# tryolabs/luminoth

Measured on NVIDIA H100. Metric: images/sec, higher is better.
Workload: dtype f32 (fp16x2-split operands on fp16 wgmma, fp32 accumulate)

## Files before the change

luminoth_b200/csrc/conv.cu:

```cuda
#include "conv.cuh"
#include <algorithm>
#include <cmath>
#include <cstdlib>
#include <cstring>
#include <map>
#include <mutex>
#include <tuple>

namespace lumi {

thread_local int g_launch_count = 0;

struct SimtArgs {
  const __half* in_hi; const __half* in_lo;
  int n, h, w, cin;
  const float* wgt; const float* scale; const float* bias;
  int kh, kw, stride, rate, pad_t, pad_l, ho, wo, cout, act;
  __half* out_hi; __half* out_lo; float* out_f32;
  const __half* res_hi; const __half* res_lo; int res_h, res_w, res_stride;
  int* overflow;
  const float* pre_scale; const float* pre_bias; __half* pre_hi; __half* pre_lo;
};

constexpr int SM_BM = 128, SM_BN = 64, SM_BK = 16;
// ... 131 lines not shown
        }
      }
    }
  }
}

void launch_conv_simt(const ConvLayer& L, const ConvIO& io, cudaStream_t st) {
  SimtArgs a;
  a.in_hi = io.in.hi; a.in_lo = io.in.lo;
  a.n = io.in.n; a.h = io.in.h; a.w = io.in.w; a.cin = io.in.c;
  LUMI_REQUIRE(io.in.c == L.cin, "conv_simt: channel mismatch");
  a.wgt = L.w_f32; a.scale = L.scale; a.bias = L.bias;
  a.kh = L.kh; a.kw = L.kw; a.stride = L.stride; a.rate = L.rate;
  a.pad_t = io.pad_t; a.pad_l = io.pad_l; a.ho = io.ho; a.wo = io.wo; a.cout = L.cout; a.act = L.act;
  a.out_hi = io.out.hi; a.out_lo = io.out.lo; a.out_f32 = io.out_f32;
  a.res_hi = io.res.hi; a.res_lo = io.res.lo; a.res_h = io.res.h; a.res_w = io.res.w; a.res_stride = io.res_stride;
  a.overflow = io.overflow_flag;
  a.pre_scale = io.pre_scale; a.pre_bias = io.pre_bias; a.pre_hi = io.pre.hi; a.pre_lo = io.pre.lo;
  LUMI_REQUIRE(!io.pre.hi || (!io.out_f32 && io.pre_scale && io.pre_bias), "conv_simt: bad pre-activation output");
  long M = (long)a.n * a.ho * a.wo;
  if (M == 0) return;
  dim3 grid((unsigned)cdiv64(M, SM_BM), (unsigned)cdiv(L.cout, SM_BN));
  if (io.pre.hi) conv_simt_kernel<true><<<grid, 256, 0, st>>>(a);
  else conv_simt_kernel<false><<<grid, 256, 0, st>>>(a);
  count_launch();
  LUMI_CUDA_CHECK(cudaGetLastError());
}

struct TcArgs {
  CUtensorMap tm_a_hi, tm_a_lo, tm_b_hi, tm_b_lo;
  CUtensorMap tm_o_hi, tm_o_lo, tm_r_hi, tm_r_lo;
  CUtensorMap tm_p_hi, tm_p_lo;
  const float* pre_scale; const float* pre_bias;
  __half* pre_hi; __half* pre_lo;
  const float* scale; const float* bias;
  __half* out_hi; __half* out_lo; float* out_f32;
  const __half* res_hi; const __half* res_lo;
  int res_h, res_w, res_stride;
  int n, ho, wo, cin, cout;
  int kh, kw, rate, pad_t, pad_l, act;
  int nb, th, tw;
  int tiles_w, tiles_h, tiles_n;
  int n_tiles;
  int stride;
  int* overflow;
  int sk_mode;
  float* sk_partials;
  int* sk_flags;
  int sk_epoch;
};

struct TcItem { int tile, k0, k1; };
struct TcSched {
  int mode, total_tiles, n_iters, t, bid, nblk;
  long long u, u_end;
  __device__ TcSched(int mode_, int total_tiles_, int n_iters_, int bid_, int nblk_)
      : mode(mode_), total_tiles(total_tiles_), n_iters(n_iters_), bid(bid_), nblk(nblk_) {
    t = bid;
    const long long U = (long long)total_tiles * n_iters;
    u = U * bid / nblk;
    u_end = U * (bid + 1) / nblk;
  }
  __device__ static long long range_end(int unit, int total_tiles, int n_iters, int nblk_) {
    return (long long)total_tiles * n_iters * (unit + 1) / nblk_;
  }
  __device__ bool next(TcItem& it) {
    if (!mode) {
      if (t >= total_tiles) return false;
      it.tile = t; it.k0 = 0; it.k1 = n_iters;
      t += nblk;
      return true;
    }
    if (u >= u_end) return false;
    it.tile = (int)(u / n_iters);
    it.k0 = (int)(u - (long long)it.tile * n_iters);
    const long long rem = u_end - u;
    it.k1 = (rem < (long long)(n_iters - it.k0)) ? it.k0 + (int)rem : n_iters;
    u += it.k1 - it.k0;
    return true;
  }
};

constexpr int TC_A_BYTES = 128 * 128;
constexpr int TC_HALO_TW = 8;
constexpr int TC_HALO_PITCH = 2048;
constexpr int TC_HALO_ROWS = 16 + 2;
constexpr int TC_HALO_PLANE_BYTES = TC_HALO_ROWS * TC_HALO_PITCH;

template <int BN, int STAGES, int NCWG = 2, bool PAIR = false, bool HALO = false, int SLOTS = 0>
struct TcCfg {
  static_assert(NCWG == 2 || NCWG == 4, "two or four consumer warpgroups");
  static_assert(!PAIR || BN == 128, "the cluster pair exists for BN = 128");
  static constexpr int WN = BN * 2 / NCWG;
  static_assert(SLOTS == 0 || (!PAIR && !HALO && WN % 64 == 0), "slot epilogue: generic kernel, whole column groups");
  static_assert(NCWG == 2 || SLOTS % 2 == 0, "four warpgroups: an even slot count");
  static constexpr int B_BYTES = BN * 128;
  static constexpr int A_STAGE_BYTES = HALO ? 0 : 2 * TC_A_BYTES;
  static constexpr int STAGE_BYTES = A_STAGE_BYTES + 2 * B_BYTES;
  static constexpr int PATCH_BYTES = HALO ? 2 * TC_HALO_PLANE_BYTES : 0;
  static constexpr int SLOT_BYTES = 2 * TC_A_BYTES;
  static constexpr int SMEM_BYTES = 2 * PATCH_BYTES + STAGES * STAGE_BYTES + SLOTS * SLOT_BYTES + 1024  +
                                    256 ;
  static_assert(SMEM_BYTES <= 232448, "shared memory per CTA");
  static constexpr int THREADS = (1 + NCWG) * 128;
  static constexpr int LAUNCH_REGS = (65536 / THREADS) / 8 * 8;
  static constexpr int PRODUCER_REGS = NCWG == 2 ? 40 : 24;
  static constexpr int CONSUMER_REGS = NCWG == 2 ? 232 : 112;
  static_assert(128 * (PRODUCER_REGS + NCWG * CONSUMER_REGS) <= THREADS * LAUNCH_REGS, "register budget of the CTA");
};

struct TcSlice { uint64_t ahi, alo, bhi, blo; uint32_t st, pb; };

template <int WN>
__device__ __forceinline__ void tc_slice_mma(float (&d)[WN / 2], const TcSlice& s) {
  wgmma_fence();
#pragma unroll
  for (int kk = 0; kk < 4; ++kk) {
    const uint64_t ko = (uint64_t)(kk * 2);
    if constexpr (WN == 128) {
      wgmma_m64n128k16_f16(d, s.ahi + ko, s.blo + ko, kk > 0 ? 1u : 0u);
      wgmma_m64n128k16_f16(d, s.alo + ko, s.bhi + ko, 1u);
    } else {
      wgmma_m64n64k16_f16(d, s.ahi + ko, s.blo + ko, kk > 0 ? 1u : 0u);
      wgmma_m64n64k16_f16(d, s.alo + ko, s.bhi + ko, 1u);
    }
  }
#pragma unroll
  for (int kk = 0; kk < 4; ++kk) {
    const uint64_t ko = (uint64_t)(kk * 2);
    if constexpr (WN == 128) wgmma_m64n128k16_f16(d, s.ahi + ko, s.bhi + ko, 1u);
    else wgmma_m64n64k16_f16(d, s.ahi + ko, s.bhi + ko, 1u);
  }
  wgmma_commit();
}

__device__ __forceinline__ bool tc_preact(__half2& h2, __half2& l2, const float* s, const float* b, int c0) {
  const float2 sc = __ldg(reinterpret_cast<const float2*>(s + c0));
  const float2 bi = __ldg(reinterpret_cast<const float2*>(b + c0));
  const float p0 = fmaxf(fmaf(__low2float(h2) + __low2float(l2), sc.x, bi.x), 0.f);
  const float p1 = fmaxf(fmaf(__high2float(h2) + __high2float(l2), sc.y, bi.y), 0.f);
  split2_f32(p0, p1, h2, l2);
  return split_overflows(p0) || split_overflows(p1);
}

template <int BN, int STAGES, int NCWG, bool PAIR, bool HALO, bool PIPE, int SLOTS, bool PRE>
__global__ void __launch_bounds__(TcCfg<BN, STAGES, NCWG, PAIR, HALO, SLOTS>::THREADS, 1)
conv_tc_kernel(const __grid_constant__ TcArgs a) {
  using Cfg = TcCfg<BN, STAGES, NCWG, PAIR, HALO, SLOTS>;
  static_assert(!PRE || !HALO, "pre-activation outputs: generic and 2-CTA kernels");
  constexpr int WN = Cfg::WN;
  constexpr int NR = WN / 2;
  constexpr int NGT = BN / 64;
  extern __shared__ uint8_t smem_raw[];
  uint8_t* smem = smem_raw + ((1024u - (smem_u32(smem_raw) & 1023u)) & 1023u);
  uint8_t* patch = smem;
  uint8_t* stages = smem + 2 * Cfg::PATCH_BYTES;
  uint8_t* slots = stages + STAGES * Cfg::STAGE_BYTES;
  uint64_t* full_bar = reinterpret_cast<uint64_t*>(slots + SLOTS * Cfg::SLOT_BYTES);
  uint64_t* empty_bar = full_bar + STAGES;
  uint64_t* patch_full_bar = empty_bar + STAGES;
  uint64_t* patch_empty_bar = patch_full_bar + 2;
  uint64_t* slot_full_bar = patch_empty_bar + 2;
  uint64_t* slot_empty_bar = slot_full_bar + SLOTS;

  const int rank = PAIR ? (int)cluster_ctarank() : 0;
  const int sched_id = PAIR ? (int)(blockIdx.x >> 1) : (int)blockIdx.x;
  const int sched_n = PAIR ? (int)(gridDim.x >> 1) : (int)gridDim.x;
  const int wg = threadIdx.x >> 7;
  const int m_tiles = a.tiles_w * a.tiles_h * a.tiles_n;
  const int total_tiles = (PAIR ? (m_tiles + 1) / 2 : m_tiles) * a.n_tiles;
  const int rows_valid = a.nb * a.th * a.tw;
  const int cchunks = a.cin >> 6;
  const int n_iters = a.kh * a.kw * cchunks;

  if (threadIdx.x == 0) {
    for (int s = 0; s < STAGES; ++s) { mbar_init(&full_bar[s], 1); mbar_init(&empty_bar[s], (PAIR ? 2 : 1) * NCWG); }
    for (int s = 0; s < 2; ++s) { mbar_init(&patch_full_bar[s], 1); mbar_init(&patch_empty_bar[s], NCWG); }
    for (int s = 0; s < SLOTS; ++s) { mbar_init(&slot_full_bar[s], 1); mbar_init(&slot_empty_bar[s], 1); }
    fence_mbar_init();
    tma_prefetch_desc(&a.tm_a_hi); tma_prefetch_desc(&a.tm_a_lo);
    tma_prefetch_desc(&a.tm_b_hi); tma_prefetch_desc(&a.tm_b_lo);
    if (SLOTS) {
      tma_prefetch_desc(&a.tm_o_hi); tma_prefetch_desc(&a.tm_o_lo);
      if (a.res_hi) { tma_prefetch_desc(&a.tm_r_hi); tma_prefetch_desc(&a.tm_r_lo); }
      if (PRE && a.out_hi) { tma_prefetch_desc(&a.tm_p_hi); tma_prefetch_desc(&a.tm_p_lo); }
    }
  }
  if (PAIR) cluster_sync_all();
  else __syncthreads();

  if (wg == 0) {
    setmaxnreg_dec<Cfg::PRODUCER_REGS>();
    if (threadIdx.x == 0) {
      const uint32_t stage_tx = (HALO ? 0u : 2u * (uint32_t)rows_valid * 128u) + 2u * (uint32_t)Cfg::B_BYTES;
      const uint32_t patch_tx = 2u * (uint32_t)(a.th + 2) * (uint32_t)((TC_HALO_TW + 2) * 128);
      const uint32_t res_tx = 2u * (uint32_t)rows_valid * 128u;
      uint32_t git = 0, gpatch = 0, gslot = 0;
      TcSched sched(a.sk_mode, total_tiles, n_iters, sched_id, sched_n);
      TcItem item;
      while (sched.next(item)) {
        const int t = item.tile;
        const int nt = t % a.n_tiles, mt = PAIR ? 2 * (t / a.n_tiles) + rank : t / a.n_tiles;
        const int x0 = (mt % a.tiles_w) * a.tw, y0 = ((mt / a.tiles_w) % a.tiles_h) * a.th;
        const int img0 = (mt / (a.tiles_w * a.tiles_h)) * a.nb, n0 = nt * BN;
        int patch_cc = -1;
        for (int k = item.k0; k < item.k1; ++k, ++git) {
          const int tap = HALO ? k % 9 : k / cchunks, cc = HALO ? k / 9 : k - tap * cchunks;
          const int r = tap / a.kw, s = tap % a.kw;
          const int iy = y0 * a.stride + r * a.rate - a.pad_t, ix = x0 * a.stride + s * a.rate - a.pad_l;
          if (HALO && cc != patch_cc) {
            patch_cc = cc;
            const uint32_t pb = gpatch & 1u;
            mbar_wait(&patch_empty_bar[pb], ((gpatch >> 1) & 1u) ^ 1u);
            uint8_t* pbase = patch + pb * Cfg::PATCH_BYTES;
            mbar_arrive_expect_tx(&patch_full_bar[pb], patch_tx);
            for (int i = 0; i < a.th + 2; ++i) {
              tma_load_4d(pbase + i * TC_HALO_PITCH, &a.tm_a_hi, &patch_full_bar[pb], cc * 64, x0 - a.pad_l,
                          y0 - a.pad_t + i, img0);
              tma_load_4d(pbase + TC_HALO_PLANE_BYTES + i * TC_HALO_PITCH, &a.tm_a_lo, &patch_full_bar[pb], cc * 64,
                          x0 - a.pad_l, y0 - a.pad_t + i, img0);
            }
            ++gpatch;
          }
          const uint32_t st = git % STAGES, ph = (git / STAGES) & 1u;
          mbar_wait(&empty_bar[st], ph ^ 1u);
          uint8_t* sbase = stages + st * Cfg::STAGE_BYTES;
          const int kcol = tap * a.cin + cc * 64;
          mbar_arrive_expect_tx(&full_bar[st], stage_tx);
          if (!HALO) {
            tma_load_4d(sbase, &a.tm_a_hi, &full_bar[st], cc * 64, ix, iy, img0);
            tma_load_4d(sbase + TC_A_BYTES, &a.tm_a_lo, &full_bar[st], cc * 64, ix, iy, img0);
          }
// ... 7 lines not shown
            tma_load_2d(bbase + Cfg::B_BYTES, &a.tm_b_lo, &full_bar[st], kcol, n0);
          }
        }
        if constexpr (SLOTS > 0) {
          for (int g = 0; g < NGT && item.k0 == 0; ++g, ++gslot) {
            const uint32_t sl = gslot % SLOTS;
            mbar_wait(&slot_empty_bar[sl], ((gslot / SLOTS) & 1u) ^ 1u);
            if (a.res_hi) {
              uint8_t* sb = slots + sl * Cfg::SLOT_BYTES;
              mbar_arrive_expect_tx(&slot_full_bar[sl], res_tx);
              tma_load_4d(sb, &a.tm_r_hi, &slot_full_bar[sl], n0 + g * 64, x0 * a.res_stride, y0 * a.res_stride, img0);
              tma_load_4d(sb + TC_A_BYTES, &a.tm_r_lo, &slot_full_bar[sl], n0 + g * 64, x0 * a.res_stride,
                          y0 * a.res_stride, img0);
            } else {
              mbar_arrive(&slot_full_bar[sl]);
            }
          }
        }
      }
    }
  } else {
    setmaxnreg_inc<Cfg::CONSUMER_REGS>();
    const int c = wg - 1;
    const int ctid = threadIdx.x - 128;
    const int wrow = (c & 1) * 64, wcol = (c >> 1) * WN;
    const int lrow = ((threadIdx.x & 127) >> 5) * 16 + ((threadIdx.x & 31) >> 2);
    const int lcol = 2 * (threadIdx.x & 3);
    uint32_t git = 0, gpatch = 0;
    uint32_t gslot = 0, rel = 0;
    const bool slot_issuer = (threadIdx.x & 127) == 0 && (c & 1) == 0;
    TcSched sched(a.sk_mode, total_tiles, n_iters, sched_id, sched_n);
    TcItem item;
    while (sched.next(item)) {
      const int t = item.tile;
      const int nt = t % a.n_tiles, mt = PAIR ? 2 * (t / a.n_tiles) + rank : t / a.n_tiles;
      const int x0 = (mt % a.tiles_w) * a.tw, y0 = ((mt / a.tiles_w) % a.tiles_h) * a.th;
      const int img0 = (mt / (a.tiles_w * a.tiles_h)) * a.nb;
      const int n0 = nt * BN + wcol;

      float racc[NR];
#pragma unroll
      for (int j = 0; j < NR; ++j) racc[j] = 0.f;
      int patch_cc = -1;
      uint32_t pb = 0;
      auto acquire = [&](int k, uint32_t g) {
        TcSlice s;
        s.st = g % STAGES;
        if (HALO) {
          const int cc = k / 9, tap = k - cc * 9;
          if (cc != patch_cc) {
            patch_cc = cc;
            pb = gpatch & 1u;
            mbar_wait(&patch_full_bar[pb], (gpatch >> 1) & 1u);
            ++gpatch;
          }
          const int r = tap / 3, c3 = tap - r * 3;
          const uint32_t pa = smem_u32(patch + pb * Cfg::PATCH_BYTES) + (uint32_t)(((wrow >> 3) + r) * TC_HALO_PITCH + c3 * 128);
          s.ahi = make_sw128_kmajor_desc(pa, TC_HALO_PITCH);
          s.alo = make_sw128_kmajor_desc(pa + TC_HALO_PLANE_BYTES, TC_HALO_PITCH);
        }
        s.pb = pb;
        mbar_wait(&full_bar[s.st], (g / STAGES) & 1u);
        const uint32_t sa = smem_u32(stages + s.st * Cfg::STAGE_BYTES);
        if (!HALO) {
          s.ahi = make_sw128_kmajor_desc(sa + wrow * 128);
          s.alo = make_sw128_kmajor_desc(sa + TC_A_BYTES + wrow * 128);
        }
        s.bhi = make_sw128_kmajor_desc(sa + Cfg::A_STAGE_BYTES + wcol * 128);
        s.blo = make_sw128_kmajor_desc(sa + Cfg::A_STAGE_BYTES + Cfg::B_BYTES + wcol * 128);
        return s;
      };
      auto release = [&](int k, const TcSlice& s) {
        if ((threadIdx.x & 127) == 0) {
          mbar_arrive(&empty_bar[s.st]);
          if (PAIR) mbar_arrive_cluster(&empty_bar[s.st], (uint32_t)(rank ^ 1));
          if (HALO && (k + 1 == item.k1 || (k + 1) % 9 == 0)) mbar_arrive(&patch_empty_bar[s.pb]);
        }
      };
      auto fold = [&](float (&d)[NR]) {
        wgmma_fence_operand(d);
#pragma unroll
        for (int j = 0; j < NR; ++j) racc[j] = __fadd_rn(racc[j], d[j]);
      };
      if constexpr (PIPE) {
        const int k1 = item.k1;
        int k = item.k0;
        float d0[NR], d1[NR];
        TcSlice s0 = acquire(k, git), s1;
        tc_slice_mma<WN>(d0, s0);
        for (; k + 2 < k1; k += 2, git += 2) {
          s1 = acquire(k + 1, git + 1);
          tc_slice_mma<WN>(d1, s1);
          wgmma_wait1();
          release(k, s0);
          fold(d0);
          s0 = acquire(k + 2, git + 2);
          tc_slice_mma<WN>(d0, s0);
          wgmma_wait1();
          release(k + 1, s1);
          fold(d1);
        }
        if (k + 1 < k1) {
          s1 = acquire(k + 1, git + 1);
          tc_slice_mma<WN>(d1, s1);
          wgmma_wait1();
          release(k, s0);
          fold(d0);
          wgmma_wait0();
          release(k + 1, s1);
          fold(d1);
          git += 2;
        } else {
          wgmma_wait0();
          release(k, s0);
          fold(d0);
          git += 1;
        }
      } else {
        for (int k = item.k0; k < item.k1; ++k, ++git) {
          const TcSlice s = acquire(k, git);
          float d[NR];
          tc_slice_mma<WN>(d, s);
          wgmma_wait0();
          release(k, s);
          fold(d);
        }
      }

      if (item.k0 != 0) {
        float* wsp = a.sk_partials + (size_t)blockIdx.x * (128 * BN);
#pragma unroll
        for (int j = 0; j < NR; ++j) {
          const int row = wrow + lrow + ((j & 2) ? 8 : 0), col = wcol + (j >> 2) * 8 + lcol + (j & 1);
          wsp[col * 128 + row] = racc[j];
        }
        __threadfence();
        named_bar_sync(1, 128 * NCWG);
        if (ctid == 0)
          asm volatile("st.release.gpu.global.s32 [%0], %1;" ::"l"(a.sk_flags + blockIdx.x), "r"(a.sk_epoch) : "memory");
        continue;
      }
      if (item.k1 != n_iters) {
        const long long tile_end = (long long)(item.tile + 1) * n_iters;
        int last_unit = sched_id;
        for (int unit = sched_id + 1;; ++unit) {
          const int cta = PAIR ? 2 * unit + rank : unit;
          int seen;
          do {
            asm volatile("ld.acquire.gpu.global.s32 %0, [%1];" : "=r"(seen) : "l"(a.sk_flags + cta) : "memory");
          } while (seen != a.sk_epoch);
          const float* wsp = a.sk_partials + (size_t)cta * (128 * BN);
#pragma unroll
          for (int j = 0; j < NR; ++j) {
            const int row = wrow + lrow + ((j & 2) ? 8 : 0), col = wcol + (j >> 2) * 8 + lcol + (j & 1);
            racc[j] = __fadd_rn(racc[j], __ldcg(wsp + col * 128 + row));
          }
          last_unit = unit;
          if (TcSched::range_end(unit, total_tiles, n_iters, sched_n) >= tile_end) break;
        }
        named_bar_sync(1, 128 * NCWG);
        if (ctid == 0)
          for (int unit = sched_id + 1; unit <= last_unit; ++unit)
            asm volatile("st.relaxed.gpu.global.s32 [%0], %1;" ::"l"(a.sk_flags + (PAIR ? 2 * unit + rank : unit)), "r"(0) : "memory");
      }

      if constexpr (SLOTS > 0) {
        bool row_ok[2];
// ... 210 lines not shown
struct MapKey {
  const void* p; int a, b, c, d, e, f, g, kind;
  bool operator<(const MapKey& o) const {
    return std::tie(p, a, b, c, d, e, f, g, kind) < std::tie(o.p, o.a, o.b, o.c, o.d, o.e, o.f, o.g, o.kind);
  }
};
static std::map<MapKey, CUtensorMap> g_map_cache;
static std::mutex g_map_mutex;

static CUtensorMap cached_act_map(const __half* base, int n, int h, int w, int c, int nb, int th, int tw, int stride,
                                  long pix_pitch, long row_pitch, long img_pitch, MapKind kind = MAP_LOAD) {
  std::lock_guard<std::mutex> lk(g_map_mutex);
  MapKey k{base, n, h, w, c + (int)(pix_pitch << 12), nb, th * 16 + stride, tw, kind};
  auto it = g_map_cache.find(k);
  if (it != g_map_cache.end()) return it->second;
  if (g_map_cache.size() > 4096) g_map_cache.clear();
  CUtensorMap m = make_map_act(base, n, h, w, c, nb, th, tw, stride, pix_pitch, row_pitch, img_pitch);
  g_map_cache[k] = m;
  return m;
}
static CUtensorMap cached_wgt_map(const __half* base, int rows, int kdim, int bn) {
  std::lock_guard<std::mutex> lk(g_map_mutex);
  MapKey k{base, rows, kdim, bn, -1, -1, -1, -1, MAP_LOAD};
  auto it = g_map_cache.find(k);
  if (it != g_map_cache.end()) return it->second;
  CUtensorMap m = make_map_wgt(base, rows, kdim, bn);
  g_map_cache[k] = m;
  return m;
}

static void pick_tile(int n, int ho, int wo, int& nb, int& th, int& tw) {
  double best = -1.0;
  nb = 1; th = 1; tw = 1;
  for (int w_ = 1; w_ <= 128 && w_ <= wo; ++w_) {
    int hmax = 128 / w_;
    if (hmax > ho) hmax = ho;
    for (int h_ = 1; h_ <= hmax; ++h_) {
      int b_ = 1;
      if (h_ == ho && w_ == wo) { b_ = 128 / (h_ * w_); if (b_ > n) b_ = n; if (b_ < 1) b_ = 1; }
      long tiles = (long)cdiv(n, b_) * cdiv(ho, h_) * cdiv(wo, w_);
      double eff = (double)n * ho * wo / ((double)tiles * 128.0);
      if (eff > best + 1e-9 || (eff > best - 1e-9 && w_ > tw)) { best = eff; nb = b_; th = h_; tw = w_; }
    }
  }
}

bool conv_tc_supported(const ConvLayer& L, const ConvIO& io) {
  if (!L.tc_ready) return false;
  if (L.stride != 1 && L.stride != 2) return false;
  if (L.stride == 2 && L.rate != 1) return false;
  if (L.cin % 64 != 0) return false;
  if (io.out_f32 == nullptr && (L.cout % 32) != 0) return false;
  if (io.res.hi && (L.cout % 32) != 0) return false;
  if (io.pre.hi && (io.out_f32 || !io.pre_scale || !io.pre_bias)) return false;
  return true;
}

int device_sm_count() {
  static int n[LUMI_MAX_DEVICES] = {0};
  int dev = 0;
  LUMI_CUDA_CHECK(cudaGetDevice(&dev));
  if (dev < 0 || dev >= LUMI_MAX_DEVICES) {
    int v = 0;
    LUMI_CUDA_CHECK(cudaDeviceGetAttribute(&v, cudaDevAttrMultiProcessorCount, dev));
    return v;
  }
  int v = __atomic_load_n(&n[dev], __ATOMIC_RELAXED);
  if (!v) {
    LUMI_CUDA_CHECK(cudaDeviceGetAttribute(&v, cudaDevAttrMultiProcessorCount, dev));
    __atomic_store_n(&n[dev], v, __ATOMIC_RELAXED);
  }
  return v;
}
static int sm_budget(int reserve) {
  const int n = device_sm_count();
  return (reserve > 0 && reserve < n) ? n - reserve : n;
}

void conv_workspace_create(ConvWorkspace& w) {
  int dev = 0, n = 0;
  LUMI_CUDA_CHECK(cudaGetDevice(&dev));
  LUMI_CUDA_CHECK(cudaDeviceGetAttribute(&n, cudaDevAttrMultiProcessorCount, dev));
  w.ctas = n;
  LUMI_CUDA_CHECK(cudaMalloc(&w.partials, (size_t)n * 128 * 128 * sizeof(float)));
  LUMI_CUDA_CHECK(cudaMalloc(&w.flags, (size_t)n * sizeof(int)));
  LUMI_CUDA_CHECK(cudaMemset(w.flags, 0, (size_t)n * sizeof(int)));
  w.epoch = 0;
}
void conv_workspace_free(ConvWorkspace& w) {
  cudaFree(w.partials); cudaFree(w.flags);
  w.partials = nullptr; w.flags = nullptr; w.ctas = 0;
}

template <int BN, int STAGES, int NCWG, bool PAIR, bool HALO, bool PIPE, int SLOTS, bool PRE>
static void launch_tc_cfg(const TcArgs& a, ConvWorkspace* sk, int streamk, int sm_reserve, cudaStream_t st) {
  using Cfg = TcCfg<BN, STAGES, NCWG, PAIR, HALO, SLOTS>;
  auto kernel = conv_tc_kernel<BN, STAGES, NCWG, PAIR, HALO, PIPE, SLOTS, PRE>;
  static bool attr_set[LUMI_MAX_DEVICES] = {false};
  int dev = 0;
  LUMI_CUDA_CHECK(cudaGetDevice(&dev));
  if (dev < 0 || dev >= LUMI_MAX_DEVICES || !__atomic_load_n(&attr_set[dev], __ATOMIC_ACQUIRE)) {
    LUMI_CUDA_CHECK(cudaFuncSetAttribute(kernel, cudaFuncAttributeMaxDynamicSharedMemorySize, Cfg::SMEM_BYTES));
    if (dev >= 0 && dev < LUMI_MAX_DEVICES) __atomic_store_n(&attr_set[dev], true, __ATOMIC_RELEASE);
  }
  const long m_tiles = (long)a.tiles_w * a.tiles_h * a.tiles_n;
  const long total = (PAIR ? (m_tiles + 1) / 2 : m_tiles) * a.n_tiles;
  const int sms = sm_budget(sm_reserve);
  int units_max = PAIR ? sms / 2 : sms;
  if (PAIR) {
    static int max_clusters[LUMI_MAX_DEVICES] = {0};
    int mc = (dev >= 0 && dev < LUMI_MAX_DEVICES) ? __atomic_load_n(&max_clusters[dev], __ATOMIC_RELAXED) : 0;
    if (!mc) {
      cudaLaunchConfig_t cfg;
      std::memset(&cfg, 0, sizeof(cfg));
      cfg.gridDim = dim3(2 * units_max, 1, 1);
      cfg.blockDim = dim3(Cfg::THREADS, 1, 1);
      cfg.dynamicSmemBytes = Cfg::SMEM_BYTES;
      cudaLaunchAttribute at[1];
      at[0].id = cudaLaunchAttributeClusterDimension;
      at[0].val.clusterDim.x = 2; at[0].val.clusterDim.y = 1; at[0].val.clusterDim.z = 1;
      cfg.attrs = at;
      cfg.numAttrs = 1;
      LUMI_CUDA_CHECK(cudaOccupancyMaxActiveClusters(&mc, kernel, &cfg));
      LUMI_REQUIRE(mc > 0, "conv_tc: the 2-CTA cluster kernel cannot be scheduled on this device");
      if (dev >= 0 && dev < LUMI_MAX_DEVICES) __atomic_store_n(&max_clusters[dev], mc, __ATOMIC_RELAXED);
    }
    if (units_max > mc) units_max = mc;
  }
  TcArgs args = a;
  args.sk_mode = 0;
  int units = (int)(total < units_max ? total : units_max);
  if (sk && sk->partials && streamk > 0 && sms <= sk->ctas) {
    const long n_iters = (long)a.kh * a.kw * (a.cin >> 6);
    const double waves = (double)total / units_max;
    const double eff = waves / std::ceil(waves);
    const long units_per_cta = total * n_iters / units_max;
    const bool forced = streamk >= 2 && units_per_cta >= 3;
    if (forced || (eff < 0.92 && n_iters >= 12 && units_per_cta >= 12)) {
      args.sk_mode = 1;
      args.sk_partials = sk->partials;
      args.sk_flags = sk->flags;
      args.sk_epoch = (int)(++sk->epoch & 0x7fffffff);
      units = units_max;
    }
  }
  if (PAIR) {
    cudaLaunchConfig_t cfg;
    std::memset(&cfg, 0, sizeof(cfg));
    cfg.gridDim = dim3(2 * units, 1, 1);
    cfg.blockDim = dim3(Cfg::THREADS, 1, 1);
    cfg.dynamicSmemBytes = Cfg::SMEM_BYTES;
    cfg.stream = st;
    cudaLaunchAttribute at[1];
    at[0].id = cudaLaunchAttributeClusterDimension;
    at[0].val.clusterDim.x = 2; at[0].val.clusterDim.y = 1; at[0].val.clusterDim.z = 1;
    cfg.attrs = at;
    cfg.numAttrs = 1;
    LUMI_CUDA_CHECK(cudaLaunchKernelEx(&cfg, kernel, args));
  } else {
    kernel<<<units, Cfg::THREADS, Cfg::SMEM_BYTES, st>>>(args);
  }
  count_launch();
  LUMI_CUDA_CHECK(cudaGetLastError());
}

template <int BN, int STAGES, int NCWG = 2, bool PAIR = false, bool HALO = false, int SLOTS = 0>
static void launch_tc(const TcArgs& a, const ConvIO& io, cudaStream_t st) {
  if constexpr (!HALO) {
    if (io.pre.hi) {
      if (io.pipe) launch_tc_cfg<BN, STAGES, NCWG, PAIR, HALO, true, SLOTS, true>(a, io.sk, io.streamk, io.sm_reserve, st);
      else launch_tc_cfg<BN, STAGES, NCWG, PAIR, HALO, false, SLOTS, true>(a, io.sk, io.streamk, io.sm_reserve, st);
      return;
    }
  }
  if (io.pipe) launch_tc_cfg<BN, STAGES, NCWG, PAIR, HALO, true, SLOTS, false>(a, io.sk, io.streamk, io.sm_reserve, st);
  else launch_tc_cfg<BN, STAGES, NCWG, PAIR, HALO, false, SLOTS, false>(a, io.sk, io.streamk, io.sm_reserve, st);
}

void launch_conv_tc(const ConvLayer& L, const ConvIO& io, cudaStream_t st) {
  LUMI_REQUIRE(conv_tc_supported(L, io), "conv_tc: layer not supported by the tensor-core kernel");
  LUMI_REQUIRE(io.in.c == L.cin, "conv_tc: channel mismatch");
  if ((long)io.in.n * io.ho * io.wo == 0) return;
  TcArgs a;
  std::memset(&a, 0, sizeof(a));
  int nb, th, tw;
  pick_tile(io.in.n, io.ho, io.wo, nb, th, tw);
  const int bn = (L.cout_pad % 128 == 0) ? 128 : 64;
  bool halo = false;
  if (io.halo && L.kh == 3 && L.kw == 3 && L.stride == 1 && L.rate == 1 && io.pad_t == 1 && io.pad_l == 1 &&
      !io.res.hi && !io.out_f32 && !io.pre.hi && !io.in_pix_pitch && !io.in_row_pitch && !io.in_img_pitch) {
    const int h_tiles = cdiv(io.ho, 16), h_th = cdiv(io.ho, h_tiles);
    const long std_tiles = (long)cdiv(io.in.n, nb) * cdiv(io.ho, th) * cdiv(io.wo, tw);
    const long halo_tiles = (long)io.in.n * h_tiles * cdiv(io.wo, TC_HALO_TW);
    if (halo_tiles * 100 <= std_tiles * io.halo_tiles_pct) { halo = true; nb = 1; th = h_th; tw = TC_HALO_TW; }
  }
  if (halo) {
    a.tm_a_hi = cached_act_map(io.in.hi, io.in.n, io.in.h, io.in.w, io.in.c, 1, 1, TC_HALO_TW + 2, 1, 0, 0, 0);
    a.tm_a_lo = cached_act_map(io.in.lo, io.in.n, io.in.h, io.in.w, io.in.c, 1, 1, TC_HALO_TW + 2, 1, 0, 0, 0);
  } else {
    a.tm_a_hi = cached_act_map(io.in.hi, io.in.n, io.in.h, io.in.w, io.in.c, nb, th, tw, L.stride, io.in_pix_pitch,
                               io.in_row_pitch, io.in_img_pitch);
    a.tm_a_lo = cached_act_map(io.in.lo, io.in.n, io.in.h, io.in.w, io.in.c, nb, th, tw, L.stride, io.in_pix_pitch,
                               io.in_row_pitch, io.in_img_pitch);
  }
  const long n_iters_all = (long)L.kh * L.kw * (L.cin >> 6);
  const bool pair = io.cta2 && bn == 128 && !io.out_f32 && n_iters_all >= io.cta2;
  const int kdim = L.kh * L.kw * L.cin;
  a.tm_b_hi = cached_wgt_map(L.w_hi, L.cout_pad, kdim, pair ? bn / 2 : bn);
  a.tm_b_lo = cached_wgt_map(L.w_lo, L.cout_pad, kdim, pair ? bn / 2 : bn);
  a.scale = L.scale_tc; a.bias = L.bias;
  a.out_hi = io.out.hi; a.out_lo = io.out.lo; a.out_f32 = io.out_f32;
  a.res_hi = io.res.hi; a.res_lo = io.res.lo; a.res_h = io.res.h; a.res_w = io.res.w; a.res_stride = io.res_stride;
  a.n = io.in.n; a.ho = io.ho; a.wo = io.wo; a.cin = L.cin; a.cout = L.cout;
  a.kh = L.kh; a.kw = L.kw; a.rate = L.rate; a.pad_t = io.pad_t; a.pad_l = io.pad_l; a.act = L.act;
  a.nb = nb; a.th = th; a.tw = tw;
  a.tiles_w = cdiv(io.wo, tw); a.tiles_h = cdiv(io.ho, th); a.tiles_n = cdiv(io.in.n, nb);
  a.n_tiles = L.cout_pad / bn;
  a.stride = L.stride;
  a.overflow = io.overflow_flag;
  a.pre_scale = io.pre_scale; a.pre_bias = io.pre_bias; a.pre_hi = io.pre.hi; a.pre_lo = io.pre.lo;
  if (halo) {
    if (pair) launch_tc<128, 2, 2, true, true>(a, io, st);
    else if (bn == 128) launch_tc<128, 2, 2, false, true>(a, io, st);
    else launch_tc<64, 4, 2, false, true>(a, io, st);
    return;
  }
  const bool epi16 = io.epi16 && bn == 128 && !io.out_f32 && n_iters_all <= io.epi16;
  if (pair) { launch_tc<128, 3, 2, true>(a, io, st); return; }
  if (!io.out_f32 && io.epi_tma) {
    if (io.pre.hi) {
      a.tm_p_hi = cached_act_map(io.pre.hi, io.in.n, io.ho, io.wo, L.cout, nb, th, tw, 1, 0, 0, 0, MAP_STORE);
      a.tm_p_lo = cached_act_map(io.pre.lo, io.in.n, io.ho, io.wo, L.cout, nb, th, tw, 1, 0, 0, 0, MAP_STORE);
    }
    if (io.out.hi) {
      a.tm_o_hi = cached_act_map(io.out.hi, io.in.n, io.ho, io.wo, L.cout, nb, th, tw, 1, 0, 0, 0, MAP_STORE);
      a.tm_o_lo = cached_act_map(io.out.lo, io.in.n, io.ho, io.wo, L.cout, nb, th, tw, 1, 0, 0, 0, MAP_STORE);
    } else {
      a.tm_o_hi = a.tm_p_hi;
      a.tm_o_lo = a.tm_p_lo;
    }
    if (io.res.hi) {
      a.tm_r_hi = cached_act_map(io.res.hi, io.res.n, io.res.h, io.res.w, io.res.c, nb, th, tw, io.res_stride, 0, 0, 0);
      a.tm_r_lo = cached_act_map(io.res.lo, io.res.n, io.res.h, io.res.w, io.res.c, nb, th, tw, io.res_stride, 0, 0, 0);
    }
    if (epi16) launch_tc<128, 2, 4, false, false, 2>(a, io, st);
    else if (bn == 128) launch_tc<128, 3, 2, false, false, 1>(a, io, st);
    else launch_tc<64, 3, 2, false, false, 2>(a, io, st);
    return;
  }
  if (epi16) launch_tc<128, 3, 4>(a, io, st);
  else if (bn == 128) launch_tc<128, 3>(a, io, st);
  else launch_tc<64, 4>(a, io, st);
}

void pack_conv_weights(const float* w, size_t kdim, int cout, const float* scale, __half* hi, __half* lo,
                       float* scale_tc) {
  for (int c = 0; c < cout; ++c) {
    float mx = 0.f;
    for (size_t k = 0; k < kdim; ++k) mx = std::fmax(mx, std::fabs(w[k * cout + c]));
    int e = 0;
    if (mx > 0.f && std::isfinite(mx)) {
      int ex;
      std::frexp(mx, &ex);
      e = 14 - ex;
      e = std::min(std::max(e, -CONV_PACK_EXP_MAX), CONV_PACK_EXP_MAX);
    }
    const float up = std::ldexp(1.f, e);
    for (size_t k = 0; k < kdim; ++k) {
      float v = w[k * cout + c] * up;
      __half h = __float2half_rn(v);
      __half l = __float2half_rn(v - __half2float(h));
      hi[(size_t)c * kdim + k] = h;
      lo[(size_t)c * kdim + k] = l;
    }
    scale_tc[c] = (float)((scale ? (double)scale[c] : 1.0) * std::ldexp(1.0, -e));
  }
}

void conv_layer_upload(ConvLayer& L, const float* w, const float* scale, const float* bias) {
  const size_t kdim = (size_t)L.kh * L.kw * L.cin;
  const size_t nw = kdim * L.cout;
  LUMI_CUDA_CHECK(cudaMalloc(&L.w_f32, nw * sizeof(float)));
  LUMI_CUDA_CHECK(cudaMemcpy(L.w_f32, w, nw * sizeof(float), cudaMemcpyHostToDevice));
  const int cpad = cdiv(L.cout, 128) * 128;
  std::vector<float> sc(cpad, 1.f), bi(cpad, 0.f);
  if (scale) std::memcpy(sc.data(), scale, L.cout * sizeof(float));
  if (bias) std::memcpy(bi.data(), bias, L.cout * sizeof(float));
  LUMI_CUDA_CHECK(cudaMalloc(&L.scale, cpad * sizeof(float)));
  LUMI_CUDA_CHECK(cudaMalloc(&L.bias, cpad * sizeof(float)));
  LUMI_CUDA_CHECK(cudaMemcpy(L.scale, sc.data(), cpad * sizeof(float), cudaMemcpyHostToDevice));
  LUMI_CUDA_CHECK(cudaMemcpy(L.bias, bi.data(), cpad * sizeof(float), cudaMemcpyHostToDevice));
  L.tc_ready = false;
  if (L.cin % 64 == 0 && (L.stride == 1 || L.stride == 2)) {
    L.cout_pad = cdiv(L.cout, 64) * 64;
    if (L.cout_pad > 64 && L.cout_pad % 128 != 0) L.cout_pad = cdiv(L.cout, 128) * 128;
    std::vector<__half> hi((size_t)L.cout_pad * kdim), lo((size_t)L.cout_pad * kdim);
    std::vector<float> sct(L.cout_pad, 0.f);
    std::memset(hi.data(), 0, hi.size() * sizeof(__half));
    std::memset(lo.data(), 0, lo.size() * sizeof(__half));
    pack_conv_weights(w, kdim, L.cout, sc.data(), hi.data(), lo.data(), sct.data());
    LUMI_CUDA_CHECK(cudaMalloc(&L.w_hi, hi.size() * sizeof(__half)));
    LUMI_CUDA_CHECK(cudaMalloc(&L.w_lo, lo.size() * sizeof(__half)));
    LUMI_CUDA_CHECK(cudaMemcpy(L.w_hi, hi.data(), hi.size() * sizeof(__half), cudaMemcpyHostToDevice));
    LUMI_CUDA_CHECK(cudaMemcpy(L.w_lo, lo.data(), lo.size() * sizeof(__half), cudaMemcpyHostToDevice));
    LUMI_CUDA_CHECK(cudaMalloc(&L.scale_tc, L.cout_pad * sizeof(float)));
    LUMI_CUDA_CHECK(cudaMemcpy(L.scale_tc, sct.data(), L.cout_pad * sizeof(float), cudaMemcpyHostToDevice));
    L.tc_ready = true;
  }
}

void conv_layer_free(ConvLayer& L) {
  cudaFree(L.w_f32); cudaFree(L.scale); cudaFree(L.bias);
  cudaFree(L.w_hi); cudaFree(L.w_lo); cudaFree(L.scale_tc);
  L = ConvLayer();
}

}
```

luminoth_b200/csrc/conv.cuh:

```cuda
#pragma once
#include "common.cuh"
#include <vector>

namespace lumi {

struct ConvLayer {
  int kh = 1, kw = 1, cin = 0, cout = 0;
  int stride = 1, rate = 1;
  int act = ACT_NONE;
  float* w_f32 = nullptr;
  float* scale = nullptr;
  float* bias = nullptr;
  __half* w_hi = nullptr;
  __half* w_lo = nullptr;
  float* scale_tc = nullptr;
  int cout_pad = 0;
  bool tc_ready = false;
};

struct ConvWorkspace {
  float* partials = nullptr;
  int* flags = nullptr;
  unsigned epoch = 0;
  int ctas = 0;
};
void conv_workspace_create(ConvWorkspace& w);
void conv_workspace_free(ConvWorkspace& w);
int device_sm_count();
constexpr int LUMI_MAX_DEVICES = 64;

struct ConvIO {
  Act in;
  Act out;
  float* out_f32 = nullptr;
  Act pre;
  const float* pre_scale = nullptr;
  const float* pre_bias = nullptr;
  Act res;
  int res_stride = 1;
  int pad_t = 0, pad_l = 0;
  int ho = 0, wo = 0;
  int* overflow_flag = nullptr;
  ConvWorkspace* sk = nullptr;
  int streamk = 1;
  int cta2 = 0;
  int halo = 0;
  int halo_tiles_pct = 150;
  int pipe = 1;
  int epi16 = 0;
  int epi_tma = 1;
  int sm_reserve = 0;
  long in_pix_pitch = 0, in_row_pitch = 0, in_img_pitch = 0;
};

constexpr int CONV_PACK_EXP_MAX = 126;
void pack_conv_weights(const float* w, size_t kdim, int cout, const float* scale, __half* hi, __half* lo,
                       float* scale_tc);

void conv_layer_upload(ConvLayer& L, const float* w_host, const float* scale_host, const float* bias_host);
void conv_layer_free(ConvLayer& L);

bool conv_tc_supported(const ConvLayer& L, const ConvIO& io);
void launch_conv_simt(const ConvLayer& L, const ConvIO& io, cudaStream_t st);
void launch_conv_tc(const ConvLayer& L, const ConvIO& io, cudaStream_t st);

inline void tf_same(int in, int k, int stride, int rate, int& out, int& pad_before) {
  int keff = k + (k - 1) * (rate - 1);
  out = (in + stride - 1) / stride;
  int total = (out - 1) * stride + keff - in;
  if (total < 0) total = 0;
  pad_before = total / 2;
}
inline int tf_valid(int in, int k, int stride, int rate) {
  int keff = k + (k - 1) * (rate - 1);
  return (in - keff) / stride + 1;
}

}
```

luminoth_b200/csrc/ops_api.cu:

```cuda
#include "../../include/luminoth_b200.h"
#include "conv.cuh"
#include "ops.cuh"

#include <cstdlib>
#include <memory>
#include <string>
#include <vector>

using namespace lumi;

namespace {
thread_local std::string g_op_error;

struct DevBuf {
  void* p = nullptr;
  explicit DevBuf(size_t bytes) { if (bytes) LUMI_CUDA_CHECK(cudaMalloc(&p, bytes)); }
  ~DevBuf() { cudaFree(p); }
  DevBuf(const DevBuf&) = delete;
  template <typename T> T* as() { return static_cast<T*>(p); }
};

struct ActBuf {
  DevBuf hi, lo;
  Act a;
  ActBuf(int n, int h, int w, int c) : hi((size_t)n * h * w * c * 2), lo((size_t)n * h * w * c * 2) {
    a.n = n; a.h = h; a.w = w; a.c = c; a.hi = hi.as<__half>(); a.lo = lo.as<__half>();
  }
};

int op_fail(const Error& e) { g_op_error = e.what(); return e.code; }

int op_conv2d(const float* x, int n, int h, int w, int cin, const float* wgt, int kh, int kw, int cout, int stride,
              int rate, int padding, const float* scale, const float* bias, const float* residual, int res_h,
              int res_w, int res_stride, int act, int impl, const float* pre_scale, const float* pre_bias, float* y,
              float* p, int* ho_out, int* wo_out, cudaStream_t st) {
  const bool preact = pre_scale != nullptr;
  LUMI_REQUIRE(impl >= 0 && impl <= 13, "conv2d: impl must be one of 0-13");
  ConvLayer L;
  L.kh = kh; L.kw = kw; L.cin = cin; L.cout = cout; L.stride = stride; L.rate = rate; L.act = act;
  const size_t nw = (size_t)kh * kw * cin * cout;
  std::vector<float> hw(nw), hs, hb;
  LUMI_CUDA_CHECK(cudaMemcpy(hw.data(), wgt, nw * sizeof(float), cudaMemcpyDeviceToHost));
  if (scale) { hs.resize(cout); LUMI_CUDA_CHECK(cudaMemcpy(hs.data(), scale, cout * sizeof(float), cudaMemcpyDeviceToHost)); }
  if (bias) { hb.resize(cout); LUMI_CUDA_CHECK(cudaMemcpy(hb.data(), bias, cout * sizeof(float), cudaMemcpyDeviceToHost)); }
  conv_layer_upload(L, hw.data(), scale ? hs.data() : nullptr, bias ? hb.data() : nullptr);
  struct Guard { ConvLayer& l; ~Guard() { conv_layer_free(l); } } guard{L};
  int ho, wo, pt = 0, pl = 0;
  if (padding == 1 || (padding == 2 && stride == 1)) {
    tf_same(h, kh, stride, rate, ho, pt); tf_same(w, kw, stride, rate, wo, pl);
  } else if (padding == 2) {
    const int keff = kh + (kh - 1) * (rate - 1);
    pt = pl = (keff - 1) / 2;
    ho = (h + (keff - 1) - keff) / stride + 1; wo = (w + (keff - 1) - keff) / stride + 1;
  } else {
    ho = tf_valid(h, kh, stride, rate); wo = tf_valid(w, kw, stride, rate);
  }
  LUMI_REQUIRE(ho > 0 && wo > 0, "conv2d: empty output");
  if (ho_out) *ho_out = ho;
  if (wo_out) *wo_out = wo;
  if (!y && !p) return LUMI_OK;
  LUMI_REQUIRE(preact ? (p && pre_bias) : (y && !p), "conv2d: bad output arguments");
  const bool simt = impl == 0 || impl == 13;
  const bool split = preact || impl >= 3;
  if (preact)
    LUMI_REQUIRE(simt || (impl >= 3 && impl <= 7) || impl == 12,
                 "conv2d_preact: impl must be 0 or 13 (SIMT) or one of the split-output codes 3-7, 12");
  if (split) LUMI_REQUIRE(cout % 32 == 0, "conv2d: split outputs need cout % 32 == 0");
  ActBuf in(n, h, w, cin);
  launch_f32_to_act(x, in.a, st);
  ConvIO io;
  io.in = in.a; io.pad_t = pt; io.pad_l = pl; io.ho = ho; io.wo = wo; io.out_f32 = y;
  std::unique_ptr<ActBuf> res;
  if (residual) {
    if (res_h <= 0) { res_h = ho; res_w = wo; res_stride = 1; }
    LUMI_REQUIRE((res_stride == 1 || res_stride == 2) && (ho - 1) * res_stride < res_h &&
                     (wo - 1) * res_stride < res_w,
                 "conv2d: the residual (sampling stride 1 or 2) must cover every output pixel");
    res.reset(new ActBuf(n, res_h, res_w, cout));
    launch_f32_to_act(residual, res->a, st);
    io.res = res->a; io.res_stride = res_stride;
  }
  std::unique_ptr<ActBuf> xo, po;
  std::unique_ptr<DevBuf> ps, pb;
  DevBuf ovf(sizeof(int));
  LUMI_CUDA_CHECK(cudaMemset(ovf.p, 0, sizeof(int)));
  if (split) {
    io.out_f32 = nullptr;
    io.overflow_flag = ovf.as<int>();
    if (y) { xo.reset(new ActBuf(n, ho, wo, cout)); io.out = xo->a; }
  }
  if (preact) {
    const int cpad = cdiv(cout, 128) * 128;
    std::vector<float> hv(cpad, 0.f);
    ps.reset(new DevBuf(cpad * sizeof(float)));
    pb.reset(new DevBuf(cpad * sizeof(float)));
    LUMI_CUDA_CHECK(cudaMemcpy(hv.data(), pre_scale, cout * sizeof(float), cudaMemcpyDeviceToHost));
    LUMI_CUDA_CHECK(cudaMemcpy(ps->p, hv.data(), cpad * sizeof(float), cudaMemcpyHostToDevice));
    LUMI_CUDA_CHECK(cudaMemcpy(hv.data(), pre_bias, cout * sizeof(float), cudaMemcpyDeviceToHost));
    LUMI_CUDA_CHECK(cudaMemcpy(pb->p, hv.data(), cpad * sizeof(float), cudaMemcpyHostToDevice));
    po.reset(new ActBuf(n, ho, wo, cout));
    io.pre = po->a; io.pre_scale = ps->as<float>(); io.pre_bias = pb->as<float>();
  }
  ConvWorkspace sk;
  struct SkGuard { ConvWorkspace& w; ~SkGuard() { conv_workspace_free(w); } } skg{sk};
  if (simt) {
    launch_conv_simt(L, io, st);
  } else {
    io.epi_tma = impl == 12 ? 0 : 1;
    io.epi16 = (impl == 4 || impl == 5) ? 8 : 0;
    io.cta2 = (impl == 6 || impl == 7 || impl == 10 || impl == 11) ? 1 : 0;
    io.halo = (impl >= 8 && impl <= 11) ? 1 : 0;
    io.halo_tiles_pct = 1000000;
    LUMI_REQUIRE(conv_tc_supported(L, io), "conv2d: this layer shape is not handled by the tensor-core kernel");
    if (impl == 2 || impl == 5 || impl == 7 || impl == 9 || impl == 11) {
      conv_workspace_create(sk);
      io.sk = &sk;
      io.streamk = 2;
    }
    launch_conv_tc(L, io, st);
  }
  if (xo) launch_act_to_f32(xo->a, y, st);
  if (po) launch_act_to_f32(po->a, p, st);
  int flag = 0;
  LUMI_CUDA_CHECK(cudaMemcpyAsync(&flag, ovf.p, sizeof(int), cudaMemcpyDeviceToHost, st));
  LUMI_CUDA_CHECK(cudaStreamSynchronize(st));
  if (flag) throw Error(LUMI_EOVERFLOW, "conv2d: an output exceeded the fp16x2 split range (|x| > 65504)");
  return LUMI_OK;
}
}

#define OP_BEGIN try {
#define OP_END                                           \
  }                                                      \
  catch (const Error& err) { return op_fail(err); }      \
  catch (const std::exception& ex) { g_op_error = ex.what(); return LUMI_EINVAL; }

extern "C" {

const char* lumi_op_last_error(void) { return g_op_error.c_str(); }

int lumi_op_conv2d(const float* x, int n, int h, int w, int cin, const float* wgt, int kh, int kw, int cout, int stride,
                   int rate, int padding, const float* scale, const float* bias, const float* residual, int act,
                   int impl, float* y, int* ho_out, int* wo_out, void* stream) {
  OP_BEGIN
  return op_conv2d(x, n, h, w, cin, wgt, kh, kw, cout, stride, rate, padding, scale, bias, residual, 0, 0, 1, act, impl,
                   nullptr, nullptr, y, nullptr, ho_out, wo_out, static_cast<cudaStream_t>(stream));
  OP_END
}

int lumi_op_conv2d_preact(const float* x, int n, int h, int w, int cin, const float* wgt, int kh, int kw, int cout,
                          int stride, int rate, int padding, const float* scale, const float* bias,
                          const float* residual, int act, int impl, const float* pre_scale, const float* pre_bias,
                          float* y, float* p, int* ho_out, int* wo_out, void* stream) {
  OP_BEGIN
  LUMI_REQUIRE(pre_scale && pre_bias, "conv2d_preact: pre_scale and pre_bias are required");
  return op_conv2d(x, n, h, w, cin, wgt, kh, kw, cout, stride, rate, padding, scale, bias, residual, 0, 0, 1, act, impl,
                   pre_scale, pre_bias, y, p, ho_out, wo_out, static_cast<cudaStream_t>(stream));
  OP_END
}

int lumi_op_conv2d_io(const float* x, int n, int h, int w, int cin, const float* wgt, int kh, int kw, int cout,
                      int stride, int rate, int padding, const float* scale, const float* bias, const float* residual,
                      int res_h, int res_w, int res_stride, int act, int impl, const float* pre_scale,
                      const float* pre_bias, float* y, float* p, int* ho_out, int* wo_out, void* stream) {
  OP_BEGIN
  LUMI_REQUIRE(!residual || res_h > 0, "conv2d_io: res_h and res_w are required with a residual");
  LUMI_REQUIRE(!pre_scale == !pre_bias, "conv2d_io: pre_scale and pre_bias go together");
  return op_conv2d(x, n, h, w, cin, wgt, kh, kw, cout, stride, rate, padding, scale, bias, residual, res_h, res_w,
                   res_stride, act, impl, pre_scale, pre_bias, y, p, ho_out, wo_out, static_cast<cudaStream_t>(stream));
  OP_END
}

int lumi_pack_conv_weights(const float* w, int kdim, int cout, const float* scale, uint16_t* hi, uint16_t* lo,
                           float* scale_tc) {
  OP_BEGIN
  LUMI_REQUIRE(w && hi && lo && scale_tc && kdim > 0 && cout > 0, "pack_conv_weights: bad arguments");
  static_assert(sizeof(__half) == sizeof(uint16_t), "fp16 bits");
  pack_conv_weights(w, (size_t)kdim, cout, scale, reinterpret_cast<__half*>(hi), reinterpret_cast<__half*>(lo),
                    scale_tc);
  return LUMI_OK;
  OP_END
}

int lumi_op_resize_bilinear(const void* src, int src_is_f32, int h0, int w0, float* dst, int h, int w, void* stream) {
  OP_BEGIN
  LUMI_REQUIRE(src && dst && h0 > 0 && w0 > 0 && h > 0 && w > 0, "resize_bilinear: bad arguments");
  cudaStream_t st = static_cast<cudaStream_t>(stream);
  launch_resize_bilinear(src, src_is_f32 != 0, h0, w0, dst, h, w, st);
  LUMI_CUDA_CHECK(cudaStreamSynchronize(st));
  return LUMI_OK;
  OP_END
}

int lumi_op_max_pool(const float* x, int n, int h, int w, int c, int k, int stride, int padding, float* y, void* stream) {
  OP_BEGIN
  cudaStream_t st = static_cast<cudaStream_t>(stream);
  int ho, wo, pt = 0, pl = 0;
// ... 241 lines not shown
```

Baseline: 895.1.

## Add wide 256-column output tile for tensor-core conv when tiles suffice

```diff
diff --git a/luminoth_b200/csrc/conv.cu b/luminoth_b200/csrc/conv.cu
--- a/luminoth_b200/csrc/conv.cu
+++ b/luminoth_b200/csrc/conv.cu
@@ -237,6 +237,7 @@
 };
 
 constexpr int TC_A_BYTES = 128 * 128;
+constexpr int TC_BN_MAX = 256;
 constexpr int TC_HALO_TW = 8;
 constexpr int TC_HALO_PITCH = 2048;
 constexpr int TC_HALO_ROWS = 16 + 2;
@@ -246,6 +247,7 @@
 struct TcCfg {
   static_assert(NCWG == 2 || NCWG == 4, "two or four consumer warpgroups");
   static_assert(!PAIR || BN == 128, "the cluster pair exists for BN = 128");
+  static_assert(BN != 256 || (NCWG == 2 && !HALO && SLOTS > 0), "the wide tile: generic kernel, two consumers, slots");
   static constexpr int WN = BN * 2 / NCWG;
   static_assert(SLOTS == 0 || (!PAIR && !HALO && WN % 64 == 0), "slot epilogue: generic kernel, whole column groups");
   static_assert(NCWG == 2 || SLOTS % 2 == 0, "four warpgroups: an even slot count");
@@ -303,6 +305,7 @@
 conv_tc_kernel(const __grid_constant__ TcArgs a) {
   using Cfg = TcCfg<BN, STAGES, NCWG, PAIR, HALO, SLOTS>;
   static_assert(!PRE || !HALO, "pre-activation outputs: generic and 2-CTA kernels");
+  static_assert(BN != 256 || (!PIPE && !PRE), "the wide tile: single-buffered, no pre-activation output");
   constexpr int WN = Cfg::WN;
   constexpr int NR = WN / 2;
   constexpr int NGT = BN / 64;
@@ -476,7 +479,27 @@
 #pragma unroll
         for (int j = 0; j < NR; ++j) racc[j] = __fadd_rn(racc[j], d[j]);
       };
-      if constexpr (PIPE) {
+      if constexpr (BN == 256) {
+        constexpr uint64_t HALF_B = (128 * 128) >> 4;
+        for (int k = item.k0; k < item.k1; ++k, ++git) {
+          const TcSlice s = acquire(k, git);
+          float d[NR / 2];
+          tc_slice_mma<128>(d, s);
+          wgmma_wait0();
+          wgmma_fence_operand(d);
+#pragma unroll
+          for (int j = 0; j < NR / 2; ++j) racc[j] = __fadd_rn(racc[j], d[j]);
+          TcSlice s1 = s;
+          s1.bhi += HALF_B;
+          s1.blo += HALF_B;
+          tc_slice_mma<128>(d, s1);
+          wgmma_wait0();
+          release(k, s);
+          wgmma_fence_operand(d);
+#pragma unroll
+          for (int j = 0; j < NR / 2; ++j) racc[NR / 2 + j] = __fadd_rn(racc[NR / 2 + j], d[j]);
+        }
+      } else if constexpr (PIPE) {
         const int k1 = item.k1;
         int k = item.k0;
         float d0[NR], d1[NR];
@@ -853,7 +876,7 @@
   LUMI_CUDA_CHECK(cudaGetDevice(&dev));
   LUMI_CUDA_CHECK(cudaDeviceGetAttribute(&n, cudaDevAttrMultiProcessorCount, dev));
   w.ctas = n;
-  LUMI_CUDA_CHECK(cudaMalloc(&w.partials, (size_t)n * 128 * 128 * sizeof(float)));
+  LUMI_CUDA_CHECK(cudaMalloc(&w.partials, (size_t)n * 128 * TC_BN_MAX * sizeof(float)));
   LUMI_CUDA_CHECK(cudaMalloc(&w.flags, (size_t)n * sizeof(int)));
   LUMI_CUDA_CHECK(cudaMemset(w.flags, 0, (size_t)n * sizeof(int)));
   w.epoch = 0;
@@ -956,9 +979,13 @@
   std::memset(&a, 0, sizeof(a));
   int nb, th, tw;
   pick_tile(io.in.n, io.ho, io.wo, nb, th, tw);
-  const int bn = (L.cout_pad % 128 == 0) ? 128 : 64;
+  const long n_iters_all = (long)L.kh * L.kw * (L.cin >> 6);
+  const long wide_tiles = (long)cdiv(io.in.n, nb) * cdiv(io.ho, th) * cdiv(io.wo, tw) * (L.cout_pad / 256);
+  const bool wide = io.wide && L.cout_pad % 256 == 0 && n_iters_all >= io.wide && !io.out_f32 && io.epi_tma &&
+                    !io.pre.hi && wide_tiles * 100 >= (long)sm_budget(io.sm_reserve) * io.wide_sm_pct;
+  const int bn = wide ? 256 : (L.cout_pad % 128 == 0) ? 128 : 64;
   bool halo = false;
-  if (io.halo && L.kh == 3 && L.kw == 3 && L.stride == 1 && L.rate == 1 && io.pad_t == 1 && io.pad_l == 1 &&
+  if (io.halo && !wide && L.kh == 3 && L.kw == 3 && L.stride == 1 && L.rate == 1 && io.pad_t == 1 && io.pad_l == 1 &&
       !io.res.hi && !io.out_f32 && !io.pre.hi && !io.in_pix_pitch && !io.in_row_pitch && !io.in_img_pitch) {
     const int h_tiles = cdiv(io.ho, 16), h_th = cdiv(io.ho, h_tiles);
     const long std_tiles = (long)cdiv(io.in.n, nb) * cdiv(io.ho, th) * cdiv(io.wo, tw);
@@ -974,7 +1001,6 @@
     a.tm_a_lo = cached_act_map(io.in.lo, io.in.n, io.in.h, io.in.w, io.in.c, nb, th, tw, L.stride, io.in_pix_pitch,
                                io.in_row_pitch, io.in_img_pitch);
   }
-  const long n_iters_all = (long)L.kh * L.kw * (L.cin >> 6);
   const bool pair = io.cta2 && bn == 128 && !io.out_f32 && n_iters_all >= io.cta2;
   const int kdim = L.kh * L.kw * L.cin;
   a.tm_b_hi = cached_wgt_map(L.w_hi, L.cout_pad, kdim, pair ? bn / 2 : bn);
@@ -1014,7 +1040,8 @@
       a.tm_r_hi = cached_act_map(io.res.hi, io.res.n, io.res.h, io.res.w, io.res.c, nb, th, tw, io.res_stride, 0, 0, 0);
       a.tm_r_lo = cached_act_map(io.res.lo, io.res.n, io.res.h, io.res.w, io.res.c, nb, th, tw, io.res_stride, 0, 0, 0);
     }
-    if (epi16) launch_tc<128, 2, 4, false, false, 2>(a, io, st);
+    if (wide) launch_tc_cfg<256, 2, 2, false, false, false, 1, false>(a, io.sk, io.streamk, io.sm_reserve, st);
+    else if (epi16) launch_tc<128, 2, 4, false, false, 2>(a, io, st);
     else if (bn == 128) launch_tc<128, 3, 2, false, false, 1>(a, io, st);
     else launch_tc<64, 3, 2, false, false, 2>(a, io, st);
     return;
diff --git a/luminoth_b200/csrc/conv.cuh b/luminoth_b200/csrc/conv.cuh
--- a/luminoth_b200/csrc/conv.cuh
+++ b/luminoth_b200/csrc/conv.cuh
@@ -48,6 +48,8 @@
   int halo_tiles_pct = 150;
   int pipe = 1;
   int epi16 = 0;
+  int wide = 16;
+  int wide_sm_pct = 50;
   int epi_tma = 1;
   int sm_reserve = 0;
   long in_pix_pitch = 0, in_row_pitch = 0, in_img_pitch = 0;
diff --git a/luminoth_b200/csrc/ops_api.cu b/luminoth_b200/csrc/ops_api.cu
--- a/luminoth_b200/csrc/ops_api.cu
+++ b/luminoth_b200/csrc/ops_api.cu
@@ -35,7 +35,7 @@
               int res_w, int res_stride, int act, int impl, const float* pre_scale, const float* pre_bias, float* y,
               float* p, int* ho_out, int* wo_out, cudaStream_t st) {
   const bool preact = pre_scale != nullptr;
-  LUMI_REQUIRE(impl >= 0 && impl <= 13, "conv2d: impl must be one of 0-13");
+  LUMI_REQUIRE(impl >= 0 && impl <= 15, "conv2d: impl must be one of 0-15");
   ConvLayer L;
   L.kh = kh; L.kw = kw; L.cin = cin; L.cout = cout; L.stride = stride; L.rate = rate; L.act = act;
   const size_t nw = (size_t)kh * kw * cin * cout;
@@ -111,8 +111,12 @@
     io.cta2 = (impl == 6 || impl == 7 || impl == 10 || impl == 11) ? 1 : 0;
     io.halo = (impl >= 8 && impl <= 11) ? 1 : 0;
     io.halo_tiles_pct = 1000000;
+    const bool wide = impl == 14 || impl == 15;
+    io.wide = wide ? 1 : 0;
+    io.wide_sm_pct = 0;
     LUMI_REQUIRE(conv_tc_supported(L, io), "conv2d: this layer shape is not handled by the tensor-core kernel");
-    if (impl == 2 || impl == 5 || impl == 7 || impl == 9 || impl == 11) {
+    if (wide) LUMI_REQUIRE(L.cout_pad % 256 == 0, "conv2d: impl 14 / 15 need C_out padded to a multiple of 256");
+    if (impl == 2 || impl == 5 || impl == 7 || impl == 9 || impl == 11 || impl == 15) {
       conv_workspace_create(sk);
       io.sk = &sk;
       io.streamk = 2;
```

After: 929.2 (median of 6 runs). 3.8% higher.
